# watsonyanghx/GAN_Lib_Tensorflow

Measured on AMD Instinct MI355X. Metric: images/sec (G+D step) SNGAN-ResNet CIFAR-10 bs=64, higher is better.
Workload: dtype bf16; 1 GPU; SNGAN ResNet CIFAR-10 32x32 bs=64 hinge: 1 G update (2x64 fakes) + 5 D updates (64 real + 64 fake) per step; global_batch=64, per_gpu_batch=64, parallelism=dp1, graphs=True, finite=True, collectives_in_graphs=False, grad_wire=fp32

## Files before the change

gan_lib_tensorflow_amd/csrc/conv_wgrad.hip:

```cpp
#include "gank_common.h"
#include "label_conv_dev.h"
#include <type_traits>
#include <stdlib.h>

#define WG_X_ZEROINS2X 16
#define WG_X_STRIDE2 32

struct WgradArgs {
  const bf16* x;
  const bf16* dy;
  float* dw;
  float* dbias;
  float* ws;
  long ws_elems;
  int N, H, W;
  int Hx, Wx;
  int Hdy, Wdy;
  int Cin, Cout;
  int ks, pad, taps;
  int M;
  int flags;
  float scale;
  int tiles_ci, tiles_co, splits, steps_per_split;
  int shw, sw;
// ... 1518 lines not shown
  return 0;
}

int gank_wgrad_dispatch(WgradArgs a, hipStream_t s) {
  GANK_REQUIRE(a.x && a.dy && a.dw, "conv_wgrad: null pointer");
  GANK_REQUIRE(a.N > 0 && a.H > 0 && a.W > 0 && a.Cin > 0 && a.Cout > 0, "conv_wgrad: bad shape");
  GANK_REQUIRE(a.ks >= 1 && a.ks <= 7, "conv_wgrad: unsupported filter size %d", a.ks);
  a.taps = a.ks * a.ks;
  a.M = a.N * a.H * a.W;
  a.sw = log2_or_neg(a.W);
  a.shw = log2_or_neg(a.H * a.W);
  GANK_REQUIRE((long)a.N * a.H * a.W < (1L << 31), "conv_wgrad: too many pixels");
  const double flops = 2.0 * a.M * (double)a.Cout * a.taps * a.Cin;
  const bool fast = (a.Cin % 8 == 0) && (a.Cout % 8 == 0);
  gank_prof_begin(1, flops, s, 2.0 * ((double)a.N * a.Hx * a.Wx * a.Cin + (double)a.N * a.Hdy * a.Wdy * a.Cout) + 4.0 * a.taps * a.Cin * a.Cout);
  int rc = -1;
  const bool same_grid = (a.flags & WG_X_STRIDE2) || wgrad_x_on_dy_grid(a);
  const bool dy_grid = (a.flags & GANK_DY_UPSAMPLE2X) || (a.Hdy == a.H && a.Wdy == a.W);
  const bool lean = fast && same_grid && dy_grid && a.sw >= 0 && a.shw >= 0 && (a.M % 64 == 0) &&
                    (long)a.N * a.Hx * a.Wx * a.Cin < (1L << 30) && (long)a.N * a.Hdy * a.Wdy * a.Cout < (1L << 30);
  if (wgrad_taps_ok(a)) rc = launch_wgrad_taps(a, s);
  if (rc < 0 && wgrad_rows_ok(a)) rc = launch_wgrad_rows(a, s);
  if (rc < 0 && lean) {
    if (a.ks == 1 && a.M <= 16384 && a.Cin >= 64 && a.Cout >= 64) rc = launch_wgrad_lean<2, 2, 1, 1>(a, s);
    else if (a.Cin >= 128 && a.Cout >= 128) rc = launch_wgrad_lean<2, 2, 2, 2>(a, s);
    else if (a.Cin >= 64 && a.Cout >= 64) rc = launch_wgrad_lean<2, 2, 1, 1>(a, s);
  }
  const bool plain = (a.flags == 0) && a.Hx == a.H && a.Wx == a.W && a.Hdy == a.H && a.Wdy == a.W &&
                     (long)a.M * (a.Cin > a.Cout ? a.Cin : a.Cout) < (1L << 30);
  if (rc < 0 && plain && a.pad == (a.ks - 1) / 2 && wgrad_narrow_stream_ok(a.N, a.H, a.W, a.Cin, a.Cout, a.ks)) {
    gank_prof_tag(1, a.ks == 3 ? "conv_wgrad_narrow_stream_kernel<3>" : "conv_wgrad_narrow_stream_kernel<1>");
    const NarrowWgArgs q = narrow_args(a.x, a.dy, a.dw, a.dbias, a.N, a.H, a.W, a.Cout, a.scale);
    rc = launch_wgrad_narrow_stream(q, a.ks, q, 0, s);
  }
  if (rc < 0 && plain && a.Cin <= 4 && a.taps * a.Cin <= 32 && a.Cout % 8 == 0) rc = launch_wgrad_packed<true>(a, s);
  if (rc < 0 && plain && a.Cout <= 4 && a.taps * a.Cout <= 32 && a.Cin % 8 == 0) {
    rc = launch_wgrad_packed<false>(a, s);
    if (rc == 0 && a.dbias) rc = gank_colsum_bf16(a.dy, a.dbias, a.M, a.Cout, a.scale, s);
  }
  if (rc >= 0) {
  } else if (fast) {
    if (a.Cin >= 128 && a.Cout >= 128) rc = launch_wgrad<2, 2, 2, 2, true, 3>(a, s);
    else if (a.Cin <= 32) rc = launch_wgrad<1, 4, 1, 1, true, 3>(a, s);
    else if (a.Cout <= 32) rc = launch_wgrad<4, 1, 1, 1, true, 3>(a, s);
    else rc = launch_wgrad<2, 2, 1, 1, true, 3>(a, s);
  } else {
    if (a.Cin >= 128 && a.Cout >= 128) rc = launch_wgrad<2, 2, 2, 2, false, 1>(a, s);
    else if (a.Cin <= 32) rc = launch_wgrad<1, 4, 1, 1, false, 1>(a, s);
    else if (a.Cout <= 32) rc = launch_wgrad<4, 1, 1, 1, false, 1>(a, s);
    else rc = launch_wgrad<2, 2, 1, 1, false, 1>(a, s);
  }
  gank_prof_end(1, s);
  return rc;
}

extern "C" long gank_conv2d_wgrad_ws_elems(int N, int H, int W, int Cin, int Cout, int ksize, int flags) {
  WgradArgs a{};
  a.N = N; a.H = H; a.W = W; a.Cin = Cin; a.Cout = Cout; a.ks = ksize; a.pad = (ksize - 1) / 2; a.flags = flags;
  const bool xup = flags & GANK_IN_UPSAMPLE2X, dyup = flags & GANK_DY_UPSAMPLE2X;
  a.Hx = xup ? H / 2 : H; a.Wx = xup ? W / 2 : W; a.Hdy = dyup ? H / 2 : H; a.Wdy = dyup ? W / 2 : W;
  a.M = N * H * W; a.sw = log2_or_neg(W); a.shw = log2_or_neg(H * W);
  if (!wgrad_taps_ok(a)) return 0;
  wgrad_taps_geometry(a);
  return a.splits > 1 ? 9L * Cin * Cout * a.splits : 0;
}

namespace { struct TapSumsRider { const int32_t* lists; float* S; int V; }; struct Dgrad1x1Rider { const void* wd; int pitch; void* dx; }; }
static int conv2d_wgrad_impl(const void* x, const void* dy, float* dw, float* dbias, float* ws, long ws_elems, int N, int H, int W, int Cin, int Cout,
                             int ksize, int flags, float scale, float* slab_ws, long slab_elems, gank_slab_job* job, void* stream,
                             const TapSumsRider* rider = nullptr, const Dgrad1x1Rider* d1 = nullptr);
extern "C" int gank_conv2d_wgrad(const void* x, const void* dy, float* dw, float* dbias, float* ws, long ws_elems, int N,
                                 int H, int W, int Cin, int Cout, int ksize, int flags, float scale, void* stream) {
  return conv2d_wgrad_impl(x, dy, dw, dbias, ws, ws_elems, N, H, W, Cin, Cout, ksize, flags, scale, nullptr, 0, nullptr, stream);
}
extern "C" long gank_conv2d_wgrad_slab_elems(int N, int H, int W, int Cin, int Cout, int ksize, int flags) {
  const long dw_elems = (long)ksize * ksize * Cin * Cout;
  const long taps_ws = gank_conv2d_wgrad_ws_elems(N, H, W, Cin, Cout, ksize, flags);
  if (taps_ws > 0) return taps_ws;
  if (dw_elems > 65536 || (long)N * H * W < 4096) return 0;
  if (!(Cin <= 4 || Cout <= 4) || ksize * ksize * (Cin <= 4 ? Cin : Cout) > 32) return 0;
  return 256 * dw_elems;
}
extern "C" int gank_conv2d_wgrad_slab_splits(int N, int H, int W, int Cin, int Cout, int ksize, int flags) {
  WgradArgs a{};
  a.N = N; a.H = H; a.W = W; a.Cin = Cin; a.Cout = Cout; a.ks = ksize; a.pad = (ksize - 1) / 2; a.flags = flags;
  const bool xup = flags & GANK_IN_UPSAMPLE2X, dyup = flags & GANK_DY_UPSAMPLE2X;
  a.Hx = xup ? H / 2 : H; a.Wx = xup ? W / 2 : W; a.Hdy = dyup ? H / 2 : H; a.Wdy = dyup ? W / 2 : W;
  a.M = N * H * W; a.sw = log2_or_neg(W); a.shw = log2_or_neg(H * W);
  if (!wgrad_taps_ok(a)) return 0;
  wgrad_taps_geometry(a);
  return (a.splits > 1 && a.splits <= 32) ? a.splits : 0;
}
static int wgrad_slabs_rows_impl(const void* x, const void* dy, float* dw_full, float* dbias, int N, int H, int W, int Cin, int Cin_total,
                                 int Cout, int ksize, int flags, float scale, float* slab_ws, long slab_elems, gank_slab_job* job, void* stream,
                                 const TapSumsRider* rider);
extern "C" int gank_conv2d_wgrad_slabs_rows(const void* x, const void* dy, float* dw_full, float* dbias, int N, int H, int W, int Cin, int Cin_total,
                                            int Cout, int ksize, int flags, float scale, float* slab_ws, long slab_elems, gank_slab_job* job, void* stream) {
  return wgrad_slabs_rows_impl(x, dy, dw_full, dbias, N, H, W, Cin, Cin_total, Cout, ksize, flags, scale, slab_ws, slab_elems, job, stream, nullptr);
}
extern "C" int gank_conv2d_wgrad_slabs_rows_tap_sums(const void* x, const void* dy, float* dw_full, float* dbias, int N, int H, int W, int Cin, int Cin_total,
                                                     int Cout, int ksize, int flags, float scale, float* slab_ws, long slab_elems, gank_slab_job* job,
                                                     const int32_t* lists, int V, float* tap_sums_ws, void* stream) {
  GANK_REQUIRE(lists && tap_sums_ws && V > 0 && V <= 16 && Cout % 64 == 0 && H % 2 == 0 && ((H / 2) * W) % 32 == 0 && (H / 2) * W <= 128 && N <= 1024,
               "conv2d_wgrad_slabs_rows_tap_sums: unsupported geometry for the tap-sums rider");
  const TapSumsRider rider{lists, tap_sums_ws, V};
  return wgrad_slabs_rows_impl(x, dy, dw_full, dbias, N, H, W, Cin, Cin_total, Cout, ksize, flags, scale, slab_ws, slab_elems, job, stream, &rider);
}
static int wgrad_slabs_rows_impl(const void* x, const void* dy, float* dw_full, float* dbias, int N, int H, int W, int Cin, int Cin_total,
                                 int Cout, int ksize, int flags, float scale, float* slab_ws, long slab_elems, gank_slab_job* job, void* stream,
                                 const TapSumsRider* rider) {
  GANK_REQUIRE(slab_ws && job && slab_elems > 0 && dw_full && Cin_total >= Cin, "conv2d_wgrad_slabs_rows: bad arguments");
  const int splits = gank_conv2d_wgrad_slab_splits(N, H, W, Cin, Cout, ksize, flags);
  GANK_REQUIRE(splits > 0 && slab_elems >= (long)ksize * ksize * Cin * Cout * splits && (Cin * Cout) % 4 == 0 && ((long)Cin_total * Cout) % 4 == 0 && scale == 1.0f,
               "conv2d_wgrad_slabs_rows: this layer has no deferred slab form (gank_conv2d_wgrad_slab_splits = %d)", splits);
  *job = gank_slab_job{nullptr, dw_full, (long)ksize * ksize * Cin * Cout, (long)ksize * ksize * Cin * Cout, 0, scale, 0, 0, 0};
  if (conv2d_wgrad_impl(x, dy, dw_full, dbias, nullptr, 0, N, H, W, Cin, Cout, ksize, flags, scale, slab_ws, slab_elems, job, stream, rider)) return 1;
  GANK_REQUIRE(job->nslabs > 0, "conv2d_wgrad_slabs_rows: the launch did not leave its reduction to the job");
  job->out_run = (long)Cin * Cout;
  job->out_pitch = (long)Cin_total * Cout;
  return 0;
}
extern "C" int gank_conv2d_wgrad_slabs(const void* x, const void* dy, float* dw, float* dbias, int N, int H, int W, int Cin, int Cout, int ksize,
                                       int flags, float scale, float* slab_ws, long slab_elems, gank_slab_job* job, void* stream) {
  GANK_REQUIRE(slab_ws && job && slab_elems > 0, "conv2d_wgrad_slabs: null slab workspace / job");
  *job = gank_slab_job{nullptr, dw, (long)ksize * ksize * Cin * Cout, (long)ksize * ksize * Cin * Cout, 0, scale, 0};
  return conv2d_wgrad_impl(x, dy, dw, dbias, nullptr, 0, N, H, W, Cin, Cout, ksize, flags, scale, slab_ws, slab_elems, job, stream);
}
static int conv2d_wgrad_impl(const void* x, const void* dy, float* dw, float* dbias, float* ws, long ws_elems, int N, int H, int W, int Cin, int Cout,
                             int ksize, int flags, float scale, float* slab_ws, long slab_elems, gank_slab_job* job, void* stream,
                             const TapSumsRider* rider, const Dgrad1x1Rider* d1) {
  GANK_REQUIRE(ksize % 2 == 1, "conv2d_wgrad: even filter sizes are not on this path (ksize=%d)", ksize);
  WgradArgs a{};
  if (d1) { a.d1_wd = (const bf16*)d1->wd; a.d1_pitch = d1->pitch; a.d1_dx = (bf16*)d1->dx; }
  if (rider) { a.rider_lists = rider->lists; a.rider_S = rider->S; a.rider_V = rider->V; a.rider_blocks = rider->V * 2 * (Cout / 64); }
  a.slab_ws = slab_ws; a.slab_elems = slab_elems; a.slab_job = job;
  if (slab_ws && !ws) { ws = slab_ws; ws_elems = slab_elems; }
  a.x = (const bf16*)x; a.dy = (const bf16*)dy; a.dw = dw; a.dbias = dbias; a.ws = ws; a.ws_elems = ws_elems;
  a.N = N; a.H = H; a.W = W;
  const bool xup = flags & GANK_IN_UPSAMPLE2X, dyup = flags & GANK_DY_UPSAMPLE2X;
  GANK_REQUIRE(!(xup || dyup) || (H % 2 == 0 && W % 2 == 0), "conv2d_wgrad: 2x flags need even size");
  a.Hx = xup ? H / 2 : H; a.Wx = xup ? W / 2 : W;
  a.Hdy = dyup ? H / 2 : H; a.Wdy = dyup ? W / 2 : W;
  a.Cin = Cin; a.Cout = Cout; a.ks = ksize; a.pad = (ksize - 1) / 2;
  a.flags = flags & (GANK_IN_UPSAMPLE2X | GANK_IN_RELU | GANK_DY_UPSAMPLE2X);
  a.scale = scale;
  return gank_wgrad_dispatch(a, (hipStream_t)stream);
}

extern "C" int gank_conv2d_dgrad(const void* dy, const void* wd, const void* residual, const void* relu_ref, void* dx, int N, int H, int W, int Cin, int Cout,
                                 int ksize, int flags, float scale, void* stream);
extern "C" int gank_conv1x1_wgrad_dgrad(const void* x, const void* dy, float* dw, float* dbias, const void* wd, int wd_pitch, void* dx, int N, int H, int W,
                                        int Cin, int Cout, void* stream) {
  GANK_REQUIRE(x && dy && dw && wd && dx && N > 0 && H > 0 && W > 0, "conv1x1_wgrad_dgrad: null pointer");
  GANK_REQUIRE(Cin % 64 == 0 && Cout % 16 == 0 && Cout <= 128 && ((long)N * H * W) % 32 == 0 && wd_pitch >= Cout && wd_pitch % 8 == 0 &&
               (long)N * H * W * Cin < (1L << 31), "conv1x1_wgrad_dgrad: needs Cin %% 64 == 0, Cout %% 16 == 0, Cout <= 128, pixels %% 32 == 0 (got %d, %d, %ld)",
               Cin, Cout, (long)N * H * W);
  const Dgrad1x1Rider d1{wd, wd_pitch, dx};
  g_d1_carried = false;
  if (conv2d_wgrad_impl(x, dy, dw, dbias, nullptr, 0, N, H, W, Cin, Cout, 1, 0, 1.0f, nullptr, 0, nullptr, stream, nullptr, &d1)) return 1;
  if (g_d1_carried) return 0;
  return gank_conv2d_dgrad(dy, wd, nullptr, nullptr, dx, N, H, W, Cin, Cout, 1, 0, 1.0f, stream);
}

extern "C" int gank_conv2d_general_wgrad(const void* x, const void* dy, float* dw, float* dbias, int N, int Hx, int Wx, int Hdy, int Wdy,
                                         int Cin, int Cout, int ksize, int stride, int pad, int flags, void* stream) {
  GANK_REQUIRE(stride == 1 || stride == 2, "conv2d_general_wgrad: stride %d (1 or 2)", stride);
  GANK_REQUIRE(pad >= 0 && pad < ksize, "conv2d_general_wgrad: pad %d outside [0, ksize)", pad);
  GANK_REQUIRE(!((flags & GANK_IN_UPSAMPLE2X) && stride == 2), "conv2d_general_wgrad: upsampled input with stride 2");
  WgradArgs a{};
  a.x = (const bf16*)x; a.dy = (const bf16*)dy; a.dw = dw; a.dbias = dbias;
  a.N = N; a.H = Hdy; a.W = Wdy; a.Hx = Hx; a.Wx = Wx; a.Hdy = Hdy; a.Wdy = Wdy;
  a.Cin = Cin; a.Cout = Cout; a.ks = ksize; a.pad = pad;
  a.flags = (flags & (GANK_IN_UPSAMPLE2X | GANK_IN_RELU)) | (stride == 2 ? WG_X_STRIDE2 : 0);
  a.scale = 1.f;
  return gank_wgrad_dispatch(a, (hipStream_t)stream);
}

__global__ void wgrad_zero_kernel(float* __restrict__ p, long n4) {
  const long i = blockIdx.x * (long)blockDim.x + threadIdx.x;
  if (i < n4) reinterpret_cast<f32x4*>(p)[i] = f32x4{0.f, 0.f, 0.f, 0.f};
}
__global__ void wgrad_fold4x4_kernel(const float* __restrict__ w4, float* __restrict__ dw, long plane4) {
  const long i = blockIdx.x * (long)blockDim.x + threadIdx.x;
  if (i >= plane4) return;
  f32x4 t[16];
#pragma unroll
  for (int k = 0; k < 16; k++) t[k] = reinterpret_cast<const f32x4*>(w4)[k * plane4 + i];
#pragma unroll
  for (int a = 0; a < 3; a++)
#pragma unroll
    for (int b = 0; b < 3; b++) {
      const f32x4 v = (t[a * 4 + b] + t[a * 4 + b + 1] + t[(a + 1) * 4 + b] + t[(a + 1) * 4 + b + 1]) * 0.25f;
      reinterpret_cast<f32x4*>(dw)[(a * 3 + b) * plane4 + i] += v;
    }
}

__global__ void wgrad_cpool_fold_slabs_kernel(const float* __restrict__ ws, float* __restrict__ dw, long plane4, int splits) {
  const long i = blockIdx.x * (long)blockDim.x + threadIdx.x;
  if (i >= plane4) return;
  const int tap = blockIdx.y, ti = tap / 3, tj = tap % 3;
  f32x4 t = {0.f, 0.f, 0.f, 0.f};
  for (int sp = 0; sp < splits; sp += 2) {
    f32x4 v[8];
#pragma unroll
    for (int u = 0; u < 8; u++) {
      const int s2 = min(sp + (u >> 2), splits - 1);
      const int src = (ti + ((u >> 1) & 1)) * 4 + tj + (u & 1);
      v[u] = reinterpret_cast<const f32x4*>(ws)[((long)s2 * 16 + src) * plane4 + i];
    }
#pragma unroll
    for (int u = 0; u < 8; u++)
      if (sp + (u >> 2) < splits) { t[0] += v[u][0]; t[1] += v[u][1]; t[2] += v[u][2]; t[3] += v[u][3]; }
  }
  f32x4 o = reinterpret_cast<f32x4*>(dw)[(long)tap * plane4 + i];
  o[0] += 0.25f * t[0]; o[1] += 0.25f * t[1]; o[2] += 0.25f * t[2]; o[3] += 0.25f * t[3];
  reinterpret_cast<f32x4*>(dw)[(long)tap * plane4 + i] = o;
}

static bool wgrad_cpool_rows_ok(int N, int Hp, int Wp, int Cin, int Cout) {
  return Hp >= 8 && Wp >= 8 && log2_or_neg(Hp) >= 0 && log2_or_neg(Wp) >= 0 && Cin % 64 == 0 && Cout % 64 == 0 &&
         (long)N * 4 * Hp * Wp * Cin < (1L << 30) && (long)N * Hp * Wp * Cout < (1L << 30);
}
static void wgrad_cpool_rows_geometry(WgradArgs& a) {
  a.tiles_ci = a.Cin / 64;
  a.tiles_co = a.Cout / 64;
  const int total_steps = a.M / 64;
  const int tiles = a.tiles_ci * a.tiles_co * 4;
  int splits = WGRAD_BLOCKS / tiles;
  if (splits > total_steps / 4) splits = total_steps / 4;
  if (splits < 1) splits = 1;
  a.steps_per_split = cdiv(total_steps, splits);
  a.splits = cdiv(total_steps, a.steps_per_split);
}

extern "C" long gank_convpool3x3_wgrad_ws_elems(int N, int Hp, int Wp, int Cin, int Cout) {
  if (!wgrad_cpool_rows_ok(N, Hp, Wp, Cin, Cout)) return 16L * Cin * Cout;
  WgradArgs a{};
  a.Cin = Cin; a.Cout = Cout; a.M = N * Hp * Wp;
  wgrad_cpool_rows_geometry(a);
  return 16L * Cin * Cout * a.splits;
}

static int convpool3x3_wgrad_impl(const void* x, const void* dy, float* dw, float* dbias, float* ws16, long ws_elems, int N, int Hp, int Wp,
                                  int Cin, int Cout, int flags, gank_slab_job* job, void* stream);
extern "C" int gank_convpool3x3_wgrad(const void* x, const void* dy, float* dw, float* dbias, float* ws16, long ws_elems, int N, int Hp, int Wp,
                                      int Cin, int Cout, int flags, void* stream) {
  return convpool3x3_wgrad_impl(x, dy, dw, dbias, ws16, ws_elems, N, Hp, Wp, Cin, Cout, flags, nullptr, stream);
}
extern "C" int gank_convpool3x3_wgrad_job(const void* x, const void* dy, float* dw, float* dbias, float* ws16, long ws_elems, int N, int Hp, int Wp,
                                          int Cin, int Cout, int flags, gank_slab_job* job, void* stream) {
  GANK_REQUIRE(job, "convpool3x3_wgrad_job: null job");
  *job = gank_slab_job{nullptr, dw, 9L * Cin * Cout, 16L * Cin * Cout, 0, 0.25f, 1};
  return convpool3x3_wgrad_impl(x, dy, dw, dbias, ws16, ws_elems, N, Hp, Wp, Cin, Cout, flags, job, stream);
}
static int convpool3x3_wgrad_impl(const void* x, const void* dy, float* dw, float* dbias, float* ws16, long ws_elems, int N, int Hp, int Wp,
                                  int Cin, int Cout, int flags, gank_slab_job* job, void* stream) {
  GANK_REQUIRE(x && dy && dw && ws16, "convpool3x3_wgrad: null pointer");
  GANK_REQUIRE(Cin % 4 == 0 && Cout % 4 == 0, "convpool3x3_wgrad: channels must be multiples of 4");
  hipStream_t s = (hipStream_t)stream;
  if (wgrad_cpool_rows_ok(N, Hp, Wp, Cin, Cout)) {
    WgradArgs a{};
    a.x = (const bf16*)x; a.dy = (const bf16*)dy; a.dw = dw; a.dbias = dbias; a.ws = ws16;
    a.N = N; a.H = Hp; a.W = Wp; a.Hx = 2 * Hp; a.Wx = 2 * Wp; a.Hdy = Hp; a.Wdy = Wp;
    a.Cin = Cin; a.Cout = Cout; a.M = N * Hp * Wp;
    a.sw = log2_or_neg(Wp); a.shw = log2_or_neg(Hp * Wp);
    wgrad_cpool_rows_geometry(a);
    GANK_REQUIRE(ws_elems >= 16L * Cin * Cout * a.splits, "convpool3x3_wgrad: workspace of %ld floats, need %ld (gank_convpool3x3_wgrad_ws_elems)",
                 ws_elems, 16L * Cin * Cout * a.splits);
    gank_prof_begin(1, 2.0 * a.M * 16.0 * Cin * Cout, s, 2.0 * ((double)N * 4 * Hp * Wp * Cin + (double)a.M * Cout) + 36.0 * Cin * Cout);
    gank_prof_tag(1, (job && a.splits <= 16 && (reinterpret_cast<uintptr_t>(dw) & 15) == 0) ? "conv_wgrad_rows_kernel<1, true, 3>"
                                                                                           : "conv_wgrad_rows_kernel<1, true, 3> + wgrad_cpool_fold_slabs_kernel");
    a.scale = 1.f;
    auto kern = (flags & GANK_IN_RELU) ? conv_wgrad_rows_kernel<1, true, 3> : conv_wgrad_rows_kernel<0, true, 3>;
    a.xcd = 1;
    hipLaunchKernelGGL(kern, dim3((unsigned)(4 * a.tiles_ci * a.tiles_co * a.splits)), dim3(512), WGRAD_ROWS_LDS, s, a);
    const long plane4 = (long)Cin * Cout / 4;
    if (job && a.splits <= 16 && (reinterpret_cast<uintptr_t>(dw) & 15) == 0) {
      job->slabs = ws16;
      job->nslabs = a.splits;
    } else {
      hipLaunchKernelGGL(wgrad_cpool_fold_slabs_kernel, dim3((unsigned)cdiv(plane4, 256), 9), dim3(256), 0, s, ws16, dw, plane4, a.splits);
    }
    gank_prof_end(1, s);
    GANK_LAUNCH_OK("convpool3x3_wgrad");
    return 0;
  }
  GANK_REQUIRE(ws_elems >= 16L * Cin * Cout, "convpool3x3_wgrad: workspace of %ld floats, need %ld", ws_elems, 16L * Cin * Cout);
  const long n4 = 16L * Cin * Cout / 4;
  hipLaunchKernelGGL(wgrad_zero_kernel, dim3((unsigned)cdiv(n4, 256)), dim3(256), 0, s, ws16, n4);
  WgradArgs a{};
  a.x = (const bf16*)x; a.dy = (const bf16*)dy; a.dw = ws16; a.dbias = dbias;
  a.N = N; a.H = Hp; a.W = Wp;
  a.Hx = 2 * Hp; a.Wx = 2 * Wp; a.Hdy = Hp; a.Wdy = Wp;
  a.Cin = Cin; a.Cout = Cout; a.ks = 4; a.pad = 1;
  a.flags = WG_X_STRIDE2 | (flags & GANK_IN_RELU);
  a.scale = 1.f;
  if (gank_wgrad_dispatch(a, s)) return 1;
  const long plane4 = (long)Cin * Cout / 4;
  hipLaunchKernelGGL(wgrad_fold4x4_kernel, dim3((unsigned)cdiv(plane4, 256)), dim3(256), 0, s, ws16, dw, plane4);
  GANK_LAUNCH_OK("convpool3x3_wgrad");
  return 0;
}

__global__ __launch_bounds__(256) void wgrad_upconv_fold_slabs_kernel(const float* __restrict__ ws, float* __restrict__ dw, int Cin, int Cout, int splits) {
  __shared__ float tile[32][33];
  const int tx = threadIdx.x & 31, ty = threadIdx.x >> 5;
  const int ci0 = blockIdx.x * 32, co0 = blockIdx.y * 32;
  const int tap = blockIdx.z, t = tap / 3, sidx = tap % 3;
  const long plane = (long)Cin * Cout;
#pragma unroll
  for (int rr = 0; rr < 4; rr++) {
    const int co = co0 + ty + 8 * rr, ci = ci0 + tx;
    float acc = 0.f;
    for (int sp0 = 0; sp0 < splits; sp0 += 4) {
      float v[4][4];
#pragma unroll
      for (int u = 0; u < 4; u++) {
        const int sp = sp0 + u < splits ? sp0 + u : splits - 1;
        const float* base = ws + (long)sp * 16 * plane + (long)co * Cin + ci;
        v[u][0] = base[((2 - t) * 4 + (2 - sidx)) * plane]; v[u][1] = base[((2 - t) * 4 + (3 - sidx)) * plane];
        v[u][2] = base[((3 - t) * 4 + (2 - sidx)) * plane]; v[u][3] = base[((3 - t) * 4 + (3 - sidx)) * plane];
      }
#pragma unroll
      for (int u = 0; u < 4; u++)
        if (sp0 + u < splits) acc += (v[u][0] + v[u][1]) + (v[u][2] + v[u][3]);
    }
    tile[ty + 8 * rr][tx] = acc;
  }
  __syncthreads();
#pragma unroll
  for (int rr = 0; rr < 4; rr++) {
    const int ci = ci0 + ty + 8 * rr, co = co0 + tx;
    dw[((long)tap * Cin + ci) * Cout + co] += tile[tx][ty + 8 * rr];
  }
}

static bool wgrad_upconv_ok(int N, int H, int W, int Cin, int Cout) {
  return Cin % 64 == 0 && Cout % 64 == 0 && wgrad_cpool_rows_ok(N, H, W, Cout, Cin);
}

extern "C" long gank_upconv3x3_wgrad_ws_elems(int N, int H, int W, int Cin, int Cout) {
  if (!wgrad_upconv_ok(N, H, W, Cin, Cout)) return 0;
  WgradArgs a{};
  a.Cin = Cout; a.Cout = Cin; a.M = N * H * W;
  wgrad_cpool_rows_geometry(a);
  return 16L * Cin * Cout * a.splits;
}

extern "C" int gank_upconv3x3_wgrad(const void* x_low, const void* dy, float* dw, float* ws16, long ws_elems, int N, int H, int W, int Cin, int Cout,
                                    void* stream) {
  GANK_REQUIRE(x_low && dy && dw && ws16, "upconv3x3_wgrad: null pointer");
  GANK_REQUIRE(wgrad_upconv_ok(N, H, W, Cin, Cout), "upconv3x3_wgrad: unsupported shape (N %d, %d x %d, %d -> %d channels): gank_upconv3x3_wgrad_ws_elems returns 0 for it",
               N, H, W, Cin, Cout);
  hipStream_t s = (hipStream_t)stream;
  WgradArgs a{};
  a.x = (const bf16*)dy; a.dy = (const bf16*)x_low; a.dw = dw; a.dbias = nullptr; a.ws = ws16;
  a.N = N; a.H = H; a.W = W; a.Hx = 2 * H; a.Wx = 2 * W; a.Hdy = H; a.Wdy = W;
  a.Cin = Cout; a.Cout = Cin; a.M = N * H * W;
  a.sw = log2_or_neg(W); a.shw = log2_or_neg(H * W);
  wgrad_cpool_rows_geometry(a);
  GANK_REQUIRE(ws_elems >= 16L * Cin * Cout * a.splits, "upconv3x3_wgrad: workspace of %ld floats, need %ld (gank_upconv3x3_wgrad_ws_elems)", ws_elems,
               16L * Cin * Cout * a.splits);
  gank_prof_begin(1, 2.0 * a.M * 16.0 * Cin * Cout, s, 2.0 * ((double)a.M * Cin + 4.0 * a.M * Cout) + 36.0 * Cin * Cout);
  gank_prof_tag(1, "conv_wgrad_rows_kernel<0, true, 3> + wgrad_upconv_fold_slabs_kernel");
  a.scale = 1.f;
  a.xcd = 1;
  hipLaunchKernelGGL((conv_wgrad_rows_kernel<0, true, 3>), dim3((unsigned)(4 * a.tiles_ci * a.tiles_co * a.splits)), dim3(512), WGRAD_ROWS_LDS, s, a);
  hipLaunchKernelGGL(wgrad_upconv_fold_slabs_kernel, dim3(Cin / 32, Cout / 32, 9), dim3(256), 0, s, ws16, dw, Cin, Cout, a.splits);
  gank_prof_end(1, s);
  GANK_LAUNCH_OK("upconv3x3_wgrad");
  return 0;
}

extern "C" int gank_conv2d_wgrad_narrow_pair(const void* x0, const void* dy0, float* dw0, float* db0, int N0, int H0, int W0, int Cout0, int ks0,
                                             const void* x1, const void* dy1, float* dw1, float* db1, int N1, int H1, int W1, int Cout1, int ks1,
                                             float scale, void* stream) {
  GANK_REQUIRE(x0 && dy0 && dw0 && x1 && dy1 && dw1, "conv2d_wgrad_narrow_pair: null pointer");
  hipStream_t s = (hipStream_t)stream;
  if (wgrad_narrow_stream_ok(N0, H0, W0, 3, Cout0, ks0) && wgrad_narrow_stream_ok(N1, H1, W1, 3, Cout1, ks1)) {
    const NarrowWgArgs a0 = narrow_args(x0, dy0, dw0, db0, N0, H0, W0, Cout0, scale), a1 = narrow_args(x1, dy1, dw1, db1, N1, H1, W1, Cout1, scale);
    const double m0 = (double)a0.M, m1 = (double)a1.M;
    gank_prof_begin(1, 2.0 * (m0 * Cout0 * ks0 * ks0 * 3 + m1 * Cout1 * ks1 * ks1 * 3), s,
                    2.0 * (m0 * (3 + Cout0) + m1 * (3 + Cout1)) + 4.0 * 3 * (ks0 * ks0 * Cout0 + ks1 * ks1 * Cout1));
    gank_prof_tag(1, "conv_wgrad_narrow_stream_kernel (pair)");
    const int rc = launch_wgrad_narrow_stream(a0, ks0, a1, ks1, s);
    gank_prof_end(1, s);
    return rc;
  }
  if (gank_conv2d_wgrad(x0, dy0, dw0, db0, nullptr, 0, N0, H0, W0, 3, Cout0, ks0, 0, scale, stream)) return 1;
  return gank_conv2d_wgrad(x1, dy1, dw1, db1, nullptr, 0, N1, H1, W1, 3, Cout1, ks1, 0, scale, stream);
}

static int wgrad_batched_impl(const gank_wgrad_item* items, int count, int N, int H, int W, int Cin, int Cout, int ksize, int flags, float scale,
                              float* ws, long ws_elems, gank_slab_job* jobs, void* stream);
extern "C" int gank_conv2d_wgrad_batched(const gank_wgrad_item* items, int count, int N, int H, int W, int Cin, int Cout,
                                         int ksize, int flags, float scale, void* stream) {
  return wgrad_batched_impl(items, count, N, H, W, Cin, Cout, ksize, flags, scale, nullptr, 0, nullptr, stream);
}
static bool wgrad_batched_geometry(WgradArgs& a, int N, int H, int W, int Cin, int Cout, int ksize, int flags, float scale, bool& rows) {
  a.N = N; a.H = H; a.W = W; a.Hx = H; a.Wx = W; a.Hdy = H; a.Wdy = W;
  a.Cin = Cin; a.Cout = Cout; a.ks = ksize; a.pad = (ksize - 1) / 2; a.taps = ksize * ksize;
  a.flags = flags & GANK_IN_RELU;
  a.scale = scale;
  a.M = N * H * W; a.sw = log2_or_neg(W); a.shw = log2_or_neg(H * W);
  const bool batchable = (flags & ~GANK_IN_RELU) == 0 && Cin % 8 == 0 && Cout % 8 == 0 && Cin >= 128 && Cout >= 128 && a.sw >= 0 &&
                         a.shw >= 0 && a.M % 64 == 0 && !wgrad_taps_ok(a) && (long)a.M * (Cin > Cout ? Cin : Cout) < (1L << 30);
  rows = batchable && wgrad_rows_ok(a);
  return batchable;
}
extern "C" long gank_conv2d_wgrad_batched_ws_elems(int count, int N, int H, int W, int Cin, int Cout, int ksize, int flags) {
  if (count <= 0 || ksize != 3) return 0;
  WgradArgs a{};
  bool rows = false;
  wgrad_batched_geometry(a, N, H, W, Cin, Cout, ksize, flags, 1.f, rows);
  if (!rows) return 0;
  long total = 0;
  for (int i = 0; i < count; i += 4) {
    const int nb = count - i < 4 ? count - i : 4;
    total += (long)nb * wgrad_rows_splits(a, nb) * 9 * Cin * Cout;
  }
  return total;
}
extern "C" int gank_conv2d_wgrad_batched_slabs(const gank_wgrad_item* items, int count, int N, int H, int W, int Cin, int Cout, int ksize,
                                               int flags, float scale, float* ws, long ws_elems, gank_slab_job* jobs, void* stream) {
  GANK_REQUIRE(ws && jobs, "conv2d_wgrad_batched_slabs: null workspace / job list");
  GANK_REQUIRE(ws_elems >= gank_conv2d_wgrad_batched_ws_elems(count, N, H, W, Cin, Cout, ksize, flags) &&
               gank_conv2d_wgrad_batched_ws_elems(count, N, H, W, Cin, Cout, ksize, flags) > 0,
               "conv2d_wgrad_batched_slabs: this geometry has no slab form, or the workspace is smaller than gank_conv2d_wgrad_batched_ws_elems");
  return wgrad_batched_impl(items, count, N, H, W, Cin, Cout, ksize, flags, scale, ws, ws_elems, jobs, stream);
}
static int wgrad_batched_impl(const gank_wgrad_item* items, int count, int N, int H, int W, int Cin, int Cout, int ksize, int flags, float scale,
                              float* ws, long ws_elems, gank_slab_job* jobs, void* stream) {
  GANK_REQUIRE(items && count > 0, "conv2d_wgrad_batched: empty list");
  GANK_REQUIRE(ksize % 2 == 1, "conv2d_wgrad_batched: even filter sizes are not on this path (ksize=%d)", ksize);
  hipStream_t s = (hipStream_t)stream;
  WgradArgs a{};
  bool rows = false;
  const bool batchable = wgrad_batched_geometry(a, N, H, W, Cin, Cout, ksize, flags, scale, rows);
  long ws_used = 0;
  int i = 0;
  while (batchable && count - i >= (rows ? 1 : 2)) {
    const int nb = count - i < 4 ? count - i : 4;
    const long slab = 9L * Cin * Cout;
    const int splits = (ws && rows) ? wgrad_rows_splits(a, nb) : 0;
    for (int j = 0; j < nb; j++) {
      GANK_REQUIRE(items[i + j].x && items[i + j].dy && items[i + j].dw, "conv2d_wgrad_batched: null pointer in item %d", i + j);
      a.xs[j] = (const bf16*)items[i + j].x; a.dys[j] = (const bf16*)items[i + j].dy;
      a.dws[j] = items[i + j].dw; a.dbs[j] = items[i + j].dbias;
      a.wss[j] = nullptr;
      if (ws && rows) {
        a.wss[j] = ws + ws_used;
        jobs[i + j] = gank_slab_job{a.wss[j], items[i + j].dw, slab, slab, splits, scale, 0};
        ws_used += (long)splits * slab;
      }
    }
    for (int j = nb; j < 4; j++) a.wss[j] = nullptr;
    a.nbatch = nb;
    a.x = a.xs[0]; a.dy = a.dys[0]; a.dw = a.dws[0]; a.dbias = a.dbs[0];
    gank_prof_begin(1, 2.0 * nb * a.M * (double)Cout * a.taps * Cin, s, nb * (2.0 * a.M * ((double)Cin + Cout) + 4.0 * a.taps * Cin * Cout));
    const int rc = rows ? launch_wgrad_rows(a, s) : launch_wgrad_lean<2, 2, 2, 2>(a, s);
    gank_prof_end(1, s);
    if (rc) return rc > 0 ? rc : gank_set_error("conv2d_wgrad_batched: mode not instantiated");
    i += nb;
  }
  for (; i < count; i++)
    if (gank_conv2d_wgrad(items[i].x, items[i].dy, items[i].dw, items[i].dbias, nullptr, 0, N, H, W, Cin, Cout, ksize, flags, scale, stream)) return 1;
  return 0;
}

extern "C" int gank_deconv2d_wgrad(const void* x, const void* dy, float* df, int N, int H, int W, int Cin, int Cout,
                                   int ksize, void* stream) {
  WgradArgs a{};
  a.x = (const bf16*)dy; a.dy = (const bf16*)x; a.dw = df;
  a.N = N; a.H = H; a.W = W;
  a.Hx = 2 * H; a.Wx = 2 * W; a.Hdy = H; a.Wdy = W;
  a.Cin = Cout; a.Cout = Cin; a.ks = ksize;
  int t = ksize - 2; if (t < 0) t = 0;
  a.pad = t / 2;
  a.flags = WG_X_STRIDE2;
  a.scale = 1.f;
  return gank_wgrad_dispatch(a, (hipStream_t)stream);
}

template __global__ void conv_wgrad_rows_kernel<0, false, 1>(WgradArgs);
template __global__ void conv_wgrad_rows_kernel<1, false, 1>(WgradArgs);
template __global__ void conv_wgrad_rows_kernel<0, true, 1>(WgradArgs);
template __global__ void conv_wgrad_rows_kernel<1, true, 1>(WgradArgs);
template __global__ void conv_wgrad_rows_kernel<0, false, 2>(WgradArgs);
template __global__ void conv_wgrad_rows_kernel<1, false, 2>(WgradArgs);
template __global__ void conv_wgrad_rows_kernel<0, true, 2>(WgradArgs);
template __global__ void conv_wgrad_rows_kernel<1, true, 2>(WgradArgs);
```

Measured before the change: 61820 images/sec.

## Add dedicated upconv wgrad kernel folding 4x4 taps to 3x3 in-block

Replaces the generic rows wgrad kernel for the upsample+3x3 conv weight gradient with a dedicated kernel. Each block now covers all 16 sub-pixel taps of a 64x64 channel tile from a shared 18x18 input halo in LDS, so blocks no longer split by tap. The 4x4 to 3x3 fold happens in the epilogue through an LDS exchange between waves, which cuts the per-split workspace from 16 to 9 planes. The final kernel then only sums across splits. This reduces workspace traffic and redundant input loads, at the cost of a new split geometry and a larger LDS footprint per block.

After: 62560 images/sec (median of 6 runs). +1.2%, better.

```diff
diff --git a/gan_lib_tensorflow_amd/csrc/conv_wgrad.hip b/gan_lib_tensorflow_amd/csrc/conv_wgrad.hip
--- a/gan_lib_tensorflow_amd/csrc/conv_wgrad.hip
+++ b/gan_lib_tensorflow_amd/csrc/conv_wgrad.hip
@@ -1844,28 +1844,181 @@
   return 0;
 }
 
-__global__ __launch_bounds__(256) void wgrad_upconv_fold_slabs_kernel(const float* __restrict__ ws, float* __restrict__ dw, int Cin, int Cout, int splits) {
+constexpr int UP16_COLS = 18;
+constexpr int UP16_XSUB = 18 * UP16_COLS * 32 + 32;
+constexpr size_t WGRAD_UP16_LDS = (size_t)2 * 2 * (UP16_XSUB + SUBS) * sizeof(bf16);
+static_assert(WGRAD_UP16_LDS <= 160 * 1024, "LDS of a CU");
+static_assert(WGRAD_UP16_LDS >= (size_t)4 * 96 * 64 * sizeof(float), "the epilogue's exchange of 2 (kh) x 2 (wave_a) x 6 folded tiles");
+
+__global__ __launch_bounds__(512) void conv_wgrad_up16_kernel(WgradArgs a) {
+  constexpr int NT = 512, COLS = UP16_COLS;
+  constexpr int XCHUNKS = 18 * COLS * 8, NXC = (XCHUNKS + NT - 1) / NT;
+  extern __shared__ __attribute__((aligned(16))) char smem[];
+  bf16* sX = reinterpret_cast<bf16*>(smem);
+  bf16* sD = sX + 2 * 2 * UP16_XSUB;
+
+  const int tid = threadIdx.x, lane = tid & 63, wave = __builtin_amdgcn_readfirstlane(tid >> 6);
+  const int wave_a = wave & 1, kh = wave >> 1;
+  int bid = xcd_remap(blockIdx.x, gridDim.x);
+  const int ntile = a.tiles_co * a.tiles_ci;
+  const int split = bid / ntile; bid -= split * ntile;
+  const int tco = bid % a.tiles_co, tci = bid / a.tiles_co;
+  const int ci0 = tci * 64, co0 = tco * 64;
+
+  const int step0 = split * a.steps_per_split;
+  int nsteps = (a.M >> 6) - step0;
+  if (nsteps > a.steps_per_split) nsteps = a.steps_per_split;
+  if (nsteps <= 0) return;
+
+  constexpr int OOB = 0x7FFFFFF0;
+  const __amdgpu_buffer_rsrc_t rs_x = __builtin_amdgcn_make_buffer_rsrc(const_cast<bf16*>(a.x), 0, a.N * a.Hx * a.Wx * a.Cin * 2, 0x00020000);
+  const __amdgpu_buffer_rsrc_t rs_dy = __builtin_amdgcn_make_buffer_rsrc(const_cast<bf16*>(a.dy), 0, a.N * a.H * a.W * a.Cout * 2, 0x00020000);
+  const int pw_shift = a.sw - 3, pi_shift = a.shw - 6;
+
+  const int cc = tid & 7;
+  const int x_c = (ci0 + cc * 8) * 2;
+  int x_ry[NXC], x_rx[NXC], x_lds[NXC];
+  bool x_on[NXC];
+#pragma unroll
+  for (int j = 0; j < NXC; j++) {
+    const int q = tid + NT * j;
+    x_on[j] = q < XCHUNKS;
+    const int hp = x_on[j] ? q >> 3 : 0;
+    const int hr = hp / COLS, hx = hp % COLS;
+    x_ry[j] = hr - 1;
+    x_rx[j] = hx - 1;
+    x_lds[j] = (cc >> 2) * UP16_XSUB + (hr * COLS + (hx & 1) * (COLS / 2) + (hx >> 1)) * 32 + (cc & 3) * 8;
+  }
+  const int d_p = tid >> 3;
+  const int d_c = (co0 + cc * 8) * 2;
+  const int d_lds = (cc >> 2) * SUBS + d_p * 32 + (cc & 3) * 8;
+
+  u32x4 rX[NXC], rD;
+  const int last = nsteps - 1;
+  int cur = 0;
+  auto load_next = [&]() {
+    const int patch = step0 + cur;
+    const int n = patch >> pi_shift;
+    const int pin = patch & ((1 << pi_shift) - 1);
+    const int py0 = (pin >> pw_shift) << 3, px0 = (pin & ((1 << pw_shift) - 1)) << 3;
+#pragma unroll
+    for (int j = 0; j < NXC; j++) {
+      const int iy = 2 * py0 + x_ry[j], ix = 2 * px0 + x_rx[j];
+      const bool ok = x_on[j] && (unsigned)iy < (unsigned)a.Hx && (unsigned)ix < (unsigned)a.Wx;
+      const int off = ((n * a.Hx + iy) * a.Wx + ix) * a.Cin * 2 + x_c;
+      rX[j] = __builtin_amdgcn_raw_buffer_load_b128(rs_x, ok ? off : OOB, 0, 0);
+    }
+    const int off = ((n * a.H + py0 + (d_p >> 3)) * a.W + px0 + (d_p & 7)) * a.Cout * 2 + d_c;
+    rD = __builtin_amdgcn_raw_buffer_load_b128(rs_dy, off, 0, 0);
+    if (cur < last) cur++;
+  };
+  auto store_step = [&](int buf) {
+#pragma unroll
+    for (int j = 0; j < NXC; j++)
+      if (x_on[j]) *reinterpret_cast<u32x4*>(sX + buf * 2 * UP16_XSUB + x_lds[j]) = rX[j];
+    *reinterpret_cast<u32x4*>(sD + buf * 2 * SUBS + d_lds) = rD;
+  };
+
+  f32x16 acc[4][2];
+#pragma unroll
+  for (int t = 0; t < 4; t++)
+#pragma unroll
+    for (int b = 0; b < 2; b++)
+#pragma unroll
+      for (int e = 0; e < 16; e++) acc[t][b][e] = 0.f;
+
+  const int g = lane >> 4, li = lane & 15;
+  const int xl = ((g >> 1) * 2 * COLS + kh * COLS + (li >> 2)) * 32 + 16 * (g & 1) + 4 * (li & 3);
+  const int dl = (8 * (g >> 1) + (li >> 2)) * 32 + 16 * (g & 1) + 4 * (li & 3);
+
+  load_next();
+  store_step(0);
+  __syncthreads();
+
+  for (int s = 0; s < nsteps; s++) {
+    const int buf = s & 1;
+    load_next();
+    const bf16* pX = sX + (buf * 2 + wave_a) * UP16_XSUB + xl;
+    const bf16* pD = sD + buf * 2 * SUBS + dl;
+#pragma unroll
+    for (int kk = 0; kk < 4; kk++) {
+      bf16x8 fb[2];
+#pragma unroll
+      for (int b = 0; b < 2; b++) {
+        const s16x4 bl = lds_tr_read(pD + b * SUBS + kk * 16 * 32), bh = lds_tr_read(pD + b * SUBS + kk * 16 * 32 + 4 * 32);
+        const s16x8 tb = {bl[0], bl[1], bl[2], bl[3], bh[0], bh[1], bh[2], bh[3]};
+        fb[b] = __builtin_bit_cast(bf16x8, tb);
+      }
+#pragma unroll
+      for (int t = 0; t < 4; t++) {
+        const int o = (4 * kk * COLS + (t & 1) * (COLS / 2) + (t >> 1)) * 32;
+        const s16x4 al = lds_tr_read(pX + o), ah = lds_tr_read(pX + o + 4 * 32);
+        const s16x8 ta = {al[0], al[1], al[2], al[3], ah[0], ah[1], ah[2], ah[3]};
+        const bf16x8 fa = __builtin_bit_cast(bf16x8, ta);
+#pragma unroll
+        for (int b = 0; b < 2; b++) acc[t][b] = GANK_MFMA32(fa, fb[b], acc[t][b]);
+      }
+    }
+    if (s + 1 < nsteps) store_step(buf ^ 1);
+    __syncthreads();
+  }
+
+#pragma unroll
+  for (int b = 0; b < 2; b++) {
+    const f32x16 e0 = acc[2][b] + acc[3][b], e1 = acc[1][b] + acc[2][b], e2 = acc[0][b] + acc[1][b];
+    acc[0][b] = e0; acc[1][b] = e1; acc[2][b] = e2;
+  }
+  float* xr = reinterpret_cast<float*>(smem);
+  if (kh == 1 || kh == 2) {
+    float* mine = xr + ((kh - 1) * 2 + wave_a) * 96 * 64 + lane;
+#pragma unroll
+    for (int s = 0; s < 3; s++)
+#pragma unroll
+      for (int b = 0; b < 2; b++)
+#pragma unroll
+        for (int e = 0; e < 16; e++) mine[((s * 2 + b) * 16 + e) * 64] = acc[s][b][e];
+  }
+  __syncthreads();
+  if (kh == 2) return;
+  const int t3 = kh == 3 ? 0 : (kh == 1 ? 1 : 2);
+  const bool other_first = kh == 3;
+  const float* theirs = xr + ((kh == 0 ? 0 : 1) * 2 + wave_a) * 96 * 64 + lane;
+  const int r = lane & 31, h = lane >> 5;
+  const long plane = (long)a.Cin * a.Cout;
+#pragma unroll
+  for (int s = 0; s < 3; s++) {
+    float* dst = a.ws + ((long)split * 9 + t3 * 3 + s) * plane;
+#pragma unroll
+    for (int b = 0; b < 2; b++) {
+      const int co = co0 + b * 32 + r;
+#pragma unroll
+      for (int e = 0; e < 16; e++) {
+        const int ci = ci0 + wave_a * 32 + (e & 3) + 8 * (e >> 2) + 4 * h;
+        const float o = theirs[((s * 2 + b) * 16 + e) * 64], m = acc[s][b][e];
+        dst[(long)ci * a.Cout + co] = other_first ? o + m : m + o;
+      }
+    }
+  }
+}
+
+__global__ __launch_bounds__(256) void wgrad_upconv_sum_slabs_kernel(const float* __restrict__ ws, float* __restrict__ dw, int Cin, int Cout, int splits) {
   __shared__ float tile[32][33];
   const int tx = threadIdx.x & 31, ty = threadIdx.x >> 5;
   const int ci0 = blockIdx.x * 32, co0 = blockIdx.y * 32;
-  const int tap = blockIdx.z, t = tap / 3, sidx = tap % 3;
+  const int tap = blockIdx.z;
   const long plane = (long)Cin * Cout;
 #pragma unroll
   for (int rr = 0; rr < 4; rr++) {
     const int co = co0 + ty + 8 * rr, ci = ci0 + tx;
+    const float* base = ws + (long)tap * plane + (long)co * Cin + ci;
     float acc = 0.f;
-    for (int sp0 = 0; sp0 < splits; sp0 += 4) {
-      float v[4][4];
-#pragma unroll
-      for (int u = 0; u < 4; u++) {
-        const int sp = sp0 + u < splits ? sp0 + u : splits - 1;
-        const float* base = ws + (long)sp * 16 * plane + (long)co * Cin + ci;
-        v[u][0] = base[((2 - t) * 4 + (2 - sidx)) * plane]; v[u][1] = base[((2 - t) * 4 + (3 - sidx)) * plane];
-        v[u][2] = base[((3 - t) * 4 + (2 - sidx)) * plane]; v[u][3] = base[((3 - t) * 4 + (3 - sidx)) * plane];
-      }
-#pragma unroll
-      for (int u = 0; u < 4; u++)
-        if (sp0 + u < splits) acc += (v[u][0] + v[u][1]) + (v[u][2] + v[u][3]);
+    for (int sp0 = 0; sp0 < splits; sp0 += 8) {
+      float v[8];
+#pragma unroll
+      for (int u = 0; u < 8; u++) v[u] = base[(long)(sp0 + u < splits ? sp0 + u : splits - 1) * 9 * plane];
+#pragma unroll
+      for (int u = 0; u < 8; u++)
+        if (sp0 + u < splits) acc += v[u];
     }
     tile[ty + 8 * rr][tx] = acc;
   }
@@ -1879,14 +2032,24 @@
 
 static bool wgrad_upconv_ok(int N, int H, int W, int Cin, int Cout) {
   return Cin % 64 == 0 && Cout % 64 == 0 && wgrad_cpool_rows_ok(N, H, W, Cout, Cin);
+}
+static void wgrad_up16_geometry(WgradArgs& a) {
+  a.tiles_ci = a.Cin / 64;
+  a.tiles_co = a.Cout / 64;
+  const int total_steps = a.M / 64;
+  int splits = WGRAD_BLOCKS / (a.tiles_ci * a.tiles_co);
+  if (splits > total_steps / 4) splits = total_steps / 4;
+  if (splits < 1) splits = 1;
+  a.steps_per_split = cdiv(total_steps, splits);
+  a.splits = cdiv(total_steps, a.steps_per_split);
 }
 
 extern "C" long gank_upconv3x3_wgrad_ws_elems(int N, int H, int W, int Cin, int Cout) {
   if (!wgrad_upconv_ok(N, H, W, Cin, Cout)) return 0;
   WgradArgs a{};
   a.Cin = Cout; a.Cout = Cin; a.M = N * H * W;
-  wgrad_cpool_rows_geometry(a);
-  return 16L * Cin * Cout * a.splits;
+  wgrad_up16_geometry(a);
+  return 9L * Cin * Cout * a.splits;
 }
 
 extern "C" int gank_upconv3x3_wgrad(const void* x_low, const void* dy, float* dw, float* ws16, long ws_elems, int N, int H, int W, int Cin, int Cout,
@@ -1900,15 +2063,16 @@
   a.N = N; a.H = H; a.W = W; a.Hx = 2 * H; a.Wx = 2 * W; a.Hdy = H; a.Wdy = W;
   a.Cin = Cout; a.Cout = Cin; a.M = N * H * W;
   a.sw = log2_or_neg(W); a.shw = log2_or_neg(H * W);
-  wgrad_cpool_rows_geometry(a);
-  GANK_REQUIRE(ws_elems >= 16L * Cin * Cout * a.splits, "upconv3x3_wgrad: workspace of %ld floats, need %ld (gank_upconv3x3_wgrad_ws_elems)", ws_elems,
-               16L * Cin * Cout * a.splits);
-  gank_prof_begin(1, 2.0 * a.M * 16.0 * Cin * Cout, s, 2.0 * ((double)a.M * Cin + 4.0 * a.M * Cout) + 36.0 * Cin * Cout);
-  gank_prof_tag(1, "conv_wgrad_rows_kernel<0, true, 3> + wgrad_upconv_fold_slabs_kernel");
+  wgrad_up16_geometry(a);
+  GANK_REQUIRE(ws_elems >= 9L * Cin * Cout * a.splits, "upconv3x3_wgrad: workspace of %ld floats, need %ld (gank_upconv3x3_wgrad_ws_elems)", ws_elems,
+               9L * Cin * Cout * a.splits);
+  GANK_MAX_DYNAMIC_LDS(conv_wgrad_up16_kernel, WGRAD_UP16_LDS, "upconv3x3_wgrad");
+  gank_prof_begin(1, 2.0 * a.M * 16.0 * Cin * Cout, s, 2.0 * ((double)a.M * Cin + 4.0 * a.M * Cout) + 2.0 * 36.0 * Cin * Cout);
+  gank_prof_tag(1, "conv_wgrad_up16_kernel + wgrad_upconv_sum_slabs_kernel");
   a.scale = 1.f;
   a.xcd = 1;
-  hipLaunchKernelGGL((conv_wgrad_rows_kernel<0, true, 3>), dim3((unsigned)(4 * a.tiles_ci * a.tiles_co * a.splits)), dim3(512), WGRAD_ROWS_LDS, s, a);
-  hipLaunchKernelGGL(wgrad_upconv_fold_slabs_kernel, dim3(Cin / 32, Cout / 32, 9), dim3(256), 0, s, ws16, dw, Cin, Cout, a.splits);
+  hipLaunchKernelGGL(conv_wgrad_up16_kernel, dim3((unsigned)(a.tiles_ci * a.tiles_co * a.splits)), dim3(512), WGRAD_UP16_LDS, s, a);
+  hipLaunchKernelGGL(wgrad_upconv_sum_slabs_kernel, dim3(Cin / 32, Cout / 32, 9), dim3(256), 0, s, ws16, dw, Cin, Cout, a.splits);
   gank_prof_end(1, s);
   GANK_LAUNCH_OK("upconv3x3_wgrad");
   return 0;
```
